# ru1ven/KeypointFusion

Measured on AMD Instinct MI355X. Metric: RGB-D img/sec fwd (B=64, 256x256), higher is better.
Workload: dtype f32; 1 GPU; KPFusion-convnext-tiny, depth+RGB UNet backbones forward, B=64/GPU 256x256 f32 (BASELINE configs[1]); batch_per_gpu=64, global_batch=64, input=256x256, parallelism=dp1 (batch shards, no collective)

## Files before the change

include/kpf.h:

```cpp
#ifndef KPF_H
#define KPF_H

#ifdef __cplusplus
extern "C" {
#endif

#define KPF_OK 0
#define KPF_EINVAL (-1)
#define KPF_ELAUNCH (-2)

#define KPF_DT_F32 0
#define KPF_DT_BF16 1
#define KPF_DT_F16 2
#define KPF_DT_F32_MMA_BF16 8
#define KPF_DT_F32_MMA_F16 9

#define KPF_ACT_RELU 1u
#define KPF_ACT_GELU 2u
#define KPF_RES_ADD 4u
#define KPF_RES_GAMMA 8u
#define KPF_RELU_AFTER_RES 16u
#define KPF_ACT_LEAKY 64u
#define KPF_IN_SPLIT 128u
#define KPF_W_SPLIT 512u
// ... 11 lines not shown
  int OH, OW, N;
  int KH, KW, sh, sw, ph, pw;
  int Kp;
  int out_ld, out_coff;
  int res_ld, res_coff;
  unsigned flags;
  float w_unscale;
  int tile_cfg;
  int groups;
  long w_gstride;
} kpf_conv_desc;

int kpf_conv2d_f32(const kpf_conv_desc* d, const float* in, const float* w, const float* bias,
                   const float* pro_scale, const float* pro_shift, const float* gamma, const float* res,
                   float* out, void* stream);

int kpf_dwconv7_ln_f32(const float* x, const float* w_dw, const float* b_dw, const float* ln_w, const float* ln_b,
                       float* y, int B, int H, int W, int C, float eps, void* stream);

int kpf_convnext_mlp_f32(const float* y, const float* x, const float* w1, const float* b1, const float* w2, const float* b2,
                         const float* gamma, float* out, long M, int C, void* stream);
int kpf_convnext_mlp_supported(int C);
int kpf_convnext_mlp_split_f32(const float* y_split, const float* x, const float* w1_split, const float* b1, float w1_unscale,
                               const float* w2_split_perm, const float* b2, float w2_unscale, const float* gamma, float* out, long M,
                               int C, void* stream);
int kpf_convnext_mlp_split_supported(int C);
int kpf_convnext_mlp_h16(const void* y, const void* x, const void* w1, const float* b1, const void* w2_chunks, const float* b2,
                         const float* gamma, void* out, long M, int C, int dtype, void* stream);
int kpf_convnext_mlp_h16_supported(int C);

// ... 324 lines not shown
int kpf_track_step_f32(const float* joints, const float* center, const float* M, const float* cube, const float* cam_para, const int* pcl_count, int B, int J,
                       int frame_w, int frame_h, float expansion, long long seed_stride, double* bbox, long long* seed, int* lost, float* crop_px,
                       float* frame_px, float* cam_mm, double* bbox_used, int* status, void* stream);

int kpf_prep_annot_u16(const unsigned char* rgb, const unsigned short* depth, const int* frame_index, int F, const float* joints_mm, const float* cam32,
                       const float* center_xyz, const unsigned char* mirror, const double* cube, int B, int J, int Hs, int Ws, int x0, int y0, int H, int W, int S,
                       float* img, float* img_rgb, float* center, float* M, float* cube_out, float* cam_para, double* com, int* bounds, double* M64, float* joint,
                       float* joint_img, double* cam64, void* stream);

int kpf_prep_uncrop_mirror_f32(const float* joints, const float* center, const float* M, const float* cube, const float* cam, const unsigned char* mirror,
                               int frame_w, int B, int J, float* crop_px, float* frame_px, void* stream);

int kpf_conv_num_tile_cfgs(void);

const char* kpf_last_error(void);
#define KPF_ABI_VERSION 23
int kpf_abi_version(void);

#ifdef __cplusplus
}
#endif
#endif
```

keypointfusion_amd/csrc/kpf_conv.hip:

```cpp
#include "kpf_common.h"
#include <stdlib.h>
#include <type_traits>

namespace {

struct ConvArgs {
  const float* in;
  const float* w;
  const float* bias;
  const float* ps;
  const float* pt;
  const float* gamma;
  const float* res;
  float* out;
  int M, N, K, Kp;
  int IH, IW, Cin, in_ld, in_coff;
  int OH, OW, ohow, KH, KW, sh, sw, ph, pw;
  int out_ld, out_coff, res_ld, res_coff;
  const float* zero;
  float w_unscale;
  unsigned flags;
  int tilesN, nblk;
  int vec;
  int dbg;
  int st_policy;
  int skew;
  int groups, g_in, g_out;
  long g_w;
};

__device__ __forceinline__ ConvArgs kpf_group_args(const ConvArgs& a0) {
  ConvArgs a = a0;
  const int g = blockIdx.y;
  a.in_coff += g * a.g_in;
  a.out_coff += g * a.g_out;
  a.res_coff += g * a.g_out;
  a.w += (long)g * a.g_w;
  if (a.bias) a.bias += g * a.g_out;
  return a;
}

__device__ __forceinline__ float gelu_erf(float x) {
  const float z = fabsf(x) * 0.70710678118654752440f;
  const float t = __builtin_amdgcn_rcpf(fmaf(0.3275911f, z, 1.0f));
  float p = fmaf(1.061405429f, t, -1.453152027f);
// ... 26 lines not shown
typedef __attribute__((address_space(3))) void lds_void_t;
typedef __attribute__((address_space(1))) void gbl_void_t;

__device__ __attribute__((aligned(16))) float kpf_zero16[4] = {0.f, 0.f, 0.f, 0.f};

#ifdef KPF_DBG_TIME
__device__ unsigned long long kpf_dbg_t[8 * 8192];
#define KPF_STAMP(i) do { if (threadIdx.x == 0 && blockIdx.x < 8192) { kpf_dbg_t[8 * blockIdx.x + (i)] = __builtin_readcyclecounter(); \
    if ((i) == 0) { kpf_dbg_t[8 * blockIdx.x + 4] = __builtin_amdgcn_s_memrealtime(); kpf_dbg_t[8 * blockIdx.x + 6] = __builtin_amdgcn_s_getreg((4 << 0) | (0 << 6) | (31 << 11)) | ((unsigned long long)__builtin_amdgcn_s_getreg((20 << 0) | (0 << 6) | (3 << 11)) << 32); } \
    if ((i) == 3) kpf_dbg_t[8 * blockIdx.x + 5] = __builtin_amdgcn_s_memrealtime(); } } while (0)
#else
#define KPF_STAMP(i)
#endif
constexpr int BK = 32;

template <int TM, int TN, int WM, int WN, bool IS1X1, bool HAS_PRO, int EPI, int ARITH, int NS>
__device__ __forceinline__ void igemm_body(const ConvArgs& a) {
  constexpr bool SPLIT = ARITH == ARITH_SPLIT || ARITH == ARITH_SPLIT_W;
  constexpr bool H16 = ARITH == ARITH_BF16 || ARITH == ARITH_F16;
  using TH = typename std::conditional<ARITH == ARITH_BF16, bf16_t, f16_t>::type;
  constexpr int BM = 16 * TM * WM;
  constexpr int BN = 16 * TN * WN;
  constexpr int NW = WM * WN;
  constexpr int RPP = 8 * NW;
  constexpr int AP = (BM + RPP - 1) / RPP;
  constexpr int BP = (BN + RPP - 1) / RPP;
  constexpr bool R16 = ARITH == ARITH_R_BF16 || ARITH == ARITH_R_F16;
  constexpr bool WHOLE = NS > 2 || ARITH == ARITH_F32 || R16;
  constexpr int BMR = WHOLE ? AP * RPP : BM;
  constexpr int BNR = WHOLE ? BP * RPP : BN;
  constexpr int TILE = (BMR + BNR) * BK;
  constexpr int CNT = AP + BP;
// ... 45 lines not shown
      riy[p] = oy * a.sh - a.ph;
      rix[p] = ox * a.sw - a.pw;
      pa[p] = a.in + ((long)b * a.IH * a.IW + (long)riy[p] * a.IW + rix[p]) * a.in_ld + a.in_coff;
    } else {
      pa[p] = a.zero;
      riy[p] = -(1 << 20);
      rix[p] = 0;
    }
  }
#pragma unroll
  for (int p = 0; p < BP; ++p) {
    const int n = n0 + lr + RPP * p;
    const int nc = n < a.N ? n : a.N - 1;
    pb[p] = a.w + (long)nc * a.Kp + kc;
  }
  int s_kt = 0, s_tap = 0, s_c = 0;
  const int s_q = IS1X1 ? 0 : BK / a.Cin, s_r = IS1X1 ? 0 : BK - s_q * a.Cin;
  const int s_rcp = IS1X1 ? 0 : (65536 + a.KW - 1) / a.KW;
  if (!IS1X1) {
    s_tap = kc / a.Cin;
    s_c = kc - s_tap * a.Cin;
  }

  auto stage = [&](int kt, int buf) {
    float* As = lds + buf * TILE;
    float* Bs = As + BMR * BK;
    if (IS1X1) {
#pragma unroll
      for (int p = 0; p < AP; ++p)
        if (WHOLE || RPP * p + 8 * wave < BM)
// ... 20 lines not shown
      }
    }
#pragma unroll
    for (int p = 0; p < BP; ++p)
      if (WHOLE || RPP * p + 8 * wave < BN)
        __builtin_amdgcn_global_load_lds((gbl_void_t*)(pb[p] + kt * BK), (lds_void_t*)(Bs + (RPP * p + 8 * wave) * BK), 16, 0, 0);
  };

  const f32x4 zero4 = {0.f, 0.f, 0.f, 0.f};
  f32x4 acc[TN][TM];
#pragma unroll
  for (int i = 0; i < TN; ++i)
#pragma unroll
    for (int j = 0; j < TM; ++j) acc[i][j] = zero4;

  const int nk = a.Kp / BK;
  const int fr = lane & 15;
  const int fg = lane >> 4;
  const int rsw = (fr >> 1) & 7;

  constexpr int EPW = H16 ? 2 : 1;
  float* pro_s = lds + NS * TILE;
  float* pro_t = pro_s + a.Kp * EPW;
  if (NS <= 2) {
    stage(0, 0);
  } else {
#pragma unroll
    for (int t = 0; t < NS - 1; ++t)
      if (t < nk) stage(t, t);
  }
  if (HAS_PRO) {
// ... 22 lines not shown
        const f32x4 tp = *reinterpret_cast<const f32x4*>(pro_t + kk);
#pragma unroll
        for (int j = 0; j < TM; ++j)
#pragma unroll
          for (int e = 0; e < 4; ++e) xf[j][e] = fmaxf(fmaf(xf[j][e], sp[e], tp[e]), 0.f);
      }
    };
    auto mma = [&](int e, const f32x4(&xf)[TM], const f32x4(&wf)[TN]) {
#pragma unroll
      for (int i = 0; i < TN; ++i)
#pragma unroll
        for (int j = 0; j < TM; ++j) acc[i][j] = __builtin_amdgcn_mfma_f32_16x16x4f32(wf[i][e], xf[j][e], acc[i][j], 0, 0, 0);
    };
    f32x4 xa[TM], wa[TN], xb[TM], wb[TN];
    read_frags(0, 0, xa, wa);
    if (nk > 1) stage(1, 1);
    for (int kt = 0; kt + 1 < nk; ++kt) {
      const int cur = kt & 1;
      read_frags(cur, 1, xb, wb);
      prologue(kt, 0, xa);
#pragma unroll
      for (int e = 0; e < 4; ++e) mma(e, xa, wa);
      prologue(kt, 1, xb);
#pragma unroll
      for (int e = 0; e < 3; ++e) mma(e, xb, wb);
      __builtin_amdgcn_sched_barrier(0);
      asm volatile("s_waitcnt vmcnt(0) lgkmcnt(0)" ::: "memory");
      __builtin_amdgcn_s_barrier();
      __builtin_amdgcn_sched_barrier(0);
      read_frags(cur ^ 1, 0, xa, wa);
      stage(kt + 2 < nk ? kt + 2 : nk - 1, cur);
      mma(3, xb, wb);
      __builtin_amdgcn_sched_group_barrier(0x100, TM + TN, 0);
#pragma unroll
      for (int q = 0; q < AP + BP; ++q) {
        __builtin_amdgcn_sched_group_barrier(0x008, (TM * TN) / (AP + BP) > 0 ? (TM * TN) / (AP + BP) : 1, 0);
        __builtin_amdgcn_sched_group_barrier(0x020, 1, 0);
      }
    }
    {
      const int kt = nk - 1, cur = kt & 1;
      read_frags(cur, 1, xb, wb);
      prologue(kt, 0, xa);
#pragma unroll
      for (int e = 0; e < 4; ++e) mma(e, xa, wa);
      prologue(kt, 1, xb);
#pragma unroll
      for (int e = 0; e < 4; ++e) mma(e, xb, wb);
    }
    asm volatile("s_waitcnt vmcnt(0)" ::: "memory");
  } else
  if constexpr (NS > 2 && ARITH == ARITH_SPLIT && !HAS_PRO) {
// ... 233 lines not shown
      __syncthreads();
    }
  }

  KPF_STAMP(2);
  const unsigned fl = a.flags;
  const bool interior = (m0 + BM <= a.M) && (n0 + BN <= a.N) && a.vec && !(fl & KPF_OUT_NCHW);
  if (interior) {
    f32x4 bvv[TN], gvv[TN];
#pragma unroll
    for (int i = 0; i < TN; ++i) {
      const int n = n0 + (wn * TN + i) * 16 + fg * 4;
      bvv[i] = a.bias ? *reinterpret_cast<const f32x4*>(a.bias + n) : zero4;
      gvv[i] = (EPI == EPI_RES && (fl & KPF_RES_GAMMA)) ? *reinterpret_cast<const f32x4*>(a.gamma + n) : zero4;
    }
    constexpr bool HAS_RES = EPI == EPI_RES || EPI == EPI_GGRAD;
    constexpr bool STAGED = H16 && !HAS_RES && TN == 4;
    constexpr int RS = TN * 16 + 8;
    TH* stg = reinterpret_cast<TH*>(lds) + wave * (TM * 16) * RS;
    if constexpr (STAGED) __syncthreads();
    f32x4 rvv[HAS_RES ? TM : 1][TN];
    if (HAS_RES) {
#pragma unroll
      for (int j = 0; j < TM; ++j) {
        const long m = m0 + (wm * TM + j) * 16 + fr;
#pragma unroll
        for (int i = 0; i < TN; ++i) {
          const long o = m * a.res_ld + a.res_coff + n0 + (wn * TN + i) * 16 + fg * 4;
          if constexpr (H16) rvv[j][i] = kpf_ld4(reinterpret_cast<const TH*>(a.res) + o);
          else rvv[j][i] = *reinterpret_cast<const f32x4*>(a.res + o);
        }
// ... 4 lines not shown
      const long m = m0 + (wm * TM + j) * 16 + fr;
#pragma unroll
      for (int i = 0; i < TN; ++i) {
        const int n = n0 + (wn * TN + i) * 16 + fg * 4;
        const f32x4 bv = bvv[i], gv = gvv[i];
        f32x4 v = acc[i][j];
        if (SPLIT) {
#pragma unroll
          for (int e = 0; e < 4; ++e) v[e] *= a.w_unscale;
        }
        if (EPI == EPI_RES) {
#pragma unroll
          for (int e = 0; e < 4; ++e) {
            float y = v[e] + bv[e];
            if (fl & KPF_RES_GAMMA) y *= gv[e];
            y += rvv[HAS_RES ? j : 0][i][e];
            if (fl & KPF_RELU_AFTER_RES) y = fmaxf(y, 0.f);
            v[e] = y;
          }
        } else if (EPI == EPI_GGRAD) {
#pragma unroll
          for (int e = 0; e < 4; ++e) v[e] = (v[e] + bv[e]) * gelu_grad_erf(rvv[HAS_RES ? j : 0][i][e]);
        } else if (EPI == EPI_GELU) {
#pragma unroll
          for (int e = 0; e < 4; ++e) v[e] = gelu_of<ARITH>(v[e] + bv[e]);
        } else if (EPI == EPI_GELU2) {
          f32x4 z;
#pragma unroll
          for (int e = 0; e < 4; ++e) z[e] = v[e] + bv[e];
          if constexpr (H16) kpf_st4(reinterpret_cast<TH*>(const_cast<float*>(a.res)) + m * a.res_ld + a.res_coff + n, z);
          else STORE4(const_cast<float*>(a.res) + m * a.res_ld + a.res_coff + n, z);
// ... 88 lines not shown
        float y = (SPLIT ? acc[i][j][e] * a.w_unscale : acc[i][j][e]) + (a.bias ? a.bias[n + e] : 0.f);
        if (EPI == EPI_GELU) y = gelu_of<ARITH>(y);
        if (EPI == EPI_GELU2) {
          if constexpr (H16) {
            reinterpret_cast<TH*>(const_cast<float*>(a.res))[(long)m * a.res_ld + a.res_coff + n + e] = (TH)y;
            y = (float)(TH)y;
          } else {
            const_cast<float*>(a.res)[(long)m * a.res_ld + a.res_coff + n + e] = y;
          }
          y = gelu_exact_erf(y);
        }
        if (EPI == EPI_LIN && (fl & KPF_ACT_RELU)) y = fmaxf(y, 0.f);
        if (EPI == EPI_LIN && (fl & KPF_ACT_LEAKY)) y = fmaxf(y, 0.01f * y);
        if (EPI == EPI_RES) {
          if (fl & KPF_RES_GAMMA) y *= a.gamma[n + e];
          if constexpr (H16) y += (float)reinterpret_cast<const TH*>(a.res)[(long)m * a.res_ld + a.res_coff + n + e];
          else y += a.res[(long)m * a.res_ld + a.res_coff + n + e];
          if (fl & KPF_RELU_AFTER_RES) y = fmaxf(y, 0.f);
        }
        if (EPI == EPI_GGRAD) {
          if constexpr (H16) y *= gelu_grad_erf((float)reinterpret_cast<const TH*>(a.res)[(long)m * a.res_ld + a.res_coff + n + e]);
          else y *= gelu_grad_erf(a.res[(long)m * a.res_ld + a.res_coff + n + e]);
        }
        if (fl & KPF_OUT_NCHW) {
          a.out[((long)b * a.N + n + e) * a.ohow + pix] = y;
        } else if constexpr (H16) {
          reinterpret_cast<TH*>(a.out)[(long)m * a.out_ld + a.out_coff + n + e] = (TH)y;
        } else if (fl & KPF_OUT_SPLIT) {
          const float yc = __builtin_amdgcn_fmed3f(y, -65504.0f, 65504.0f);
          const _Float16 h = (_Float16)yc;
          _Float16* blk = reinterpret_cast<_Float16*>(a.out + (long)m * a.out_ld + a.out_coff + ((n + e) & ~31)) + ((n + e) & 31);
          blk[0] = h;
          blk[32] = (_Float16)(yc - (float)h);
        } else
          a.out[(long)m * a.out_ld + a.out_coff + n + e] = y;
      }
    }
  }
}

template <int TM, int TN, int WM, int WN, bool IS1X1, bool HAS_PRO, int EPI, int NS>
__global__ __launch_bounds__(64 * WM * WN) void igemm_f32_kernel(const ConvArgs a) {
  igemm_body<TM, TN, WM, WN, IS1X1, HAS_PRO, EPI, ARITH_F32, NS>(kpf_group_args(a));
}
template <int TM, int TN, int WM, int WN, bool IS1X1, int EPI, int ARITH>
__global__ __launch_bounds__(64 * WM * WN) void igemm_r16_kernel(const ConvArgs a) {
  igemm_body<TM, TN, WM, WN, IS1X1, false, EPI, ARITH, 2>(kpf_group_args(a));
}
template <int TM, int TN, int WM, int WN, bool IS1X1, bool HAS_PRO, int EPI, int ARITH, int NS>
__global__ __launch_bounds__(64 * WM * WN) void igemm_split_kernel(const ConvArgs a) {
  igemm_body<TM, TN, WM, WN, IS1X1, HAS_PRO, EPI, ARITH, NS>(kpf_group_args(a));
}
template <int TM, int TN, int WM, int WN, bool IS1X1, bool HAS_PRO, int EPI, int ARITH>
__global__ __launch_bounds__(64 * WM * WN, 4) void igemm_split_occ_kernel(const ConvArgs a) {
  igemm_body<TM, TN, WM, WN, IS1X1, HAS_PRO, EPI, ARITH, 1>(kpf_group_args(a));
}

template <int TM, int TN, int WM, int WN, bool IS1X1, bool HAS_PRO, int EPI, int ARITH, int NS>
// ... 31 lines not shown
  else
    kern = igemm_split_kernel<TM, TN, WM, WN, IS1X1, HAS_PRO, EPI, ARITH, NS>;
  static std::atomic<bool> lds_opt_in[KPF_MAX_DEVICES];
  if (!kpf_raise_lds_limit(reinterpret_cast<const void*>(kern), lds_opt_in)) {
    kpf_set_error("kpf_conv2d_f32: cannot raise the dynamic LDS limit");
    return KPF_ELAUNCH;
  }
  if (lds > 160 * 1024) {
    kpf_set_error("kpf_conv2d_f32: operand prologue too long for LDS (Kp=%d)", a.Kp);
    return KPF_EINVAL;
  }
  hipLaunchKernelGGL(kern, dim3(a.nblk, a.groups > 1 ? a.groups : 1), dim3(64 * WM * WN), lds, st, a);
  return kpf_check_launch("kpf_conv2d_f32");
}

template <int TM, int TN, int WM, int WN, int ARITH, int NS>
int launch_arith(ConvArgs& a, bool is1x1, hipStream_t st) {
  const bool res = a.flags & KPF_RES_ADD, gelu = a.flags & KPF_ACT_GELU;
  if (a.ps) {
    if (!is1x1 || res || gelu || ARITH == ARITH_SPLIT || (NS == 1 && (ARITH == ARITH_BF16 || ARITH == ARITH_F16))) {
      kpf_set_error("kpf_conv2d_f32: the operand prologue is only supported for 1x1 stride-1 convolutions with Cin %% 32 == 0, fp32 activations and a linear/ReLU epilogue");
      return KPF_EINVAL;
    }
    return launch_one<TM, TN, WM, WN, true, true, EPI_LIN, ARITH == ARITH_SPLIT ? ARITH_F32 : ARITH, NS>(a, st);
  }
  if (gelu) {
    if (!is1x1 || res) {
      kpf_set_error("kpf_conv2d_f32: GELU is only supported on 1x1 convolutions (Cin %% 32 == 0) without residual");
      return KPF_EINVAL;
    }
    if (a.flags & KPF_ACT_GELU_SAVE) {
      if constexpr (ARITH == ARITH_F32 && NS == 2) return launch_one<TM, TN, WM, WN, true, false, EPI_GELU2, ARITH, NS>(a, st);
      kpf_set_error("kpf_conv2d_f32: KPF_ACT_GELU_SAVE needs fp32 arithmetic");
// ... 2 lines not shown
    return launch_one<TM, TN, WM, WN, true, false, EPI_GELU, ARITH, NS>(a, st);
  }
  if (a.flags & KPF_RES_GELU_GRAD) {
    if constexpr (ARITH == ARITH_F32 && NS == 2) {
      if (a.KH == 1 && a.KW == 1 && a.sh == 1 && a.sw == 1)
        return is1x1 ? launch_one<TM, TN, WM, WN, true, false, EPI_GGRAD, ARITH, NS>(a, st) : launch_one<TM, TN, WM, WN, false, false, EPI_GGRAD, ARITH, NS>(a, st);
    }
    kpf_set_error("kpf_conv2d_f32: KPF_RES_GELU_GRAD needs a 1x1 stride-1 convolution in fp32 arithmetic");
    return KPF_EINVAL;
  }
  if (is1x1) return res ? launch_one<TM, TN, WM, WN, true, false, EPI_RES, ARITH, NS>(a, st) : launch_one<TM, TN, WM, WN, true, false, EPI_LIN, ARITH, NS>(a, st);
  return res ? launch_one<TM, TN, WM, WN, false, false, EPI_RES, ARITH, NS>(a, st) : launch_one<TM, TN, WM, WN, false, false, EPI_LIN, ARITH, NS>(a, st);
}

template <int TM, int TN, int WM, int WN, int NS_SPLIT = 2>
int launch_cfg(ConvArgs& a, bool is1x1, hipStream_t st) {
  constexpr int BM = 16 * TM * WM, BN = 16 * TN * WN;
  const int tilesM = (a.M + BM - 1) / BM;
  a.tilesN = (a.N + BN - 1) / BN;
  a.nblk = tilesM * a.tilesN;
  static const int stagger = []() { const char* e = getenv("KPF_STAGGER"); return e ? atoi(e) : 0; }();
  const long skew = (long)BM * BN * a.Kp / (128L * 5 * 2048);
  a.skew = a.nblk >= 512 ? (int)(skew < stagger ? skew : stagger) : 0;
  if constexpr ((TM == 4 && TN == 4 && WN == 2 && (WM == 4 || WM == 2)) || (TM == 2 && TN == 4 && WM == 4 && WN == 1)) {
    if ((a.flags & (KPF_MMA_BF16 | KPF_MMA_F16)) && is1x1 && !a.ps && !(a.flags & (KPF_RES_ADD | KPF_ACT_GELU | KPF_IN_SPLIT | KPF_W_SPLIT | KPF_OUT_SPLIT | KPF_OUT_NCHW))) {
      if (a.flags & KPF_MMA_BF16) return launch_one<TM, TN, WM, WN, true, false, EPI_LIN, ARITH_R_BF16, 2>(a, st);
      return launch_one<TM, TN, WM, WN, true, false, EPI_LIN, ARITH_R_F16, 2>(a, st);
    }
  }
  if (a.flags & KPF_IN_SPLIT) return launch_arith<TM, TN, WM, WN, ARITH_SPLIT, NS_SPLIT>(a, is1x1, st);
  if (a.flags & KPF_W_SPLIT) return launch_arith<TM, TN, WM, WN, ARITH_SPLIT_W, NS_SPLIT>(a, is1x1, st);
// ... 560 lines not shown
    case 1: return launch_cfg_h16<4, 3, 2, 2, 2>(a, fast1x1, pointwise, dtype, st);
    case 2: return launch_cfg_h16<2, 4, 4, 1, 2>(a, fast1x1, pointwise, dtype, st);
    case 5: return launch_cfg_h16<2, 4, 2, 2, 2>(a, fast1x1, pointwise, dtype, st);
    case 6: return occ ? launch_cfg_h16<2, 2, 2, 2, 1>(a, fast1x1, pointwise, dtype, st) : launch_cfg_h16<2, 2, 2, 2, 2>(a, fast1x1, pointwise, dtype, st);
    case 8: return launch_cfg_h16<4, 4, 4, 2, 2>(a, fast1x1, pointwise, dtype, st);
    case 20: return launch_cfg_h16<4, 4, 4, 2, 3>(a, fast1x1, pointwise, dtype, st);
    case 21: return launch_cfg_h16<4, 4, 2, 2, 3>(a, fast1x1, pointwise, dtype, st);
    case 22: return launch_cfg_h16<4, 4, 2, 2, 4>(a, fast1x1, pointwise, dtype, st);
    case 26: return launch_cfg_h16<8, 4, 2, 4, 2>(a, fast1x1, pointwise, dtype, st);
    case 41: return launch_cfg_h16<2, 2, 2, 2, 4>(a, fast1x1, pointwise, dtype, st);
    case 44: return launch_cfg_h16<2, 1, 1, 4, 8>(a, fast1x1, pointwise, dtype, st);
    default: return launch_cfg_h16<2, 1, 1, 4, 2>(a, fast1x1, pointwise, dtype, st);
  }
}
#else
extern "C" int kpf_conv2d_f32(const kpf_conv_desc* d, const float* in, const float* w, const float* bias,
                              const float* pro_scale, const float* pro_shift, const float* gamma, const float* res,
                              float* out, void* stream) {
  KPF_REQUIRE(d && in && w && out, "kpf_conv2d_f32: null pointer");
  KPF_REQUIRE(d->B > 0 && d->OH > 0 && d->OW > 0 && d->N > 0 && d->Cin > 0, "kpf_conv2d_f32: empty shape");
  KPF_REQUIRE(d->Cin % 4 == 0 && d->in_ld % 4 == 0 && d->in_coff % 4 == 0,
              "kpf_conv2d_f32: Cin/in_ld/in_coff must be multiples of 4 (got %d/%d/%d)", d->Cin, d->in_ld, d->in_coff);
  KPF_REQUIRE(d->Kp % 32 == 0 && d->Kp >= d->KH * d->KW * d->Cin, "kpf_conv2d_f32: Kp=%d must be a multiple of 32 and >= K=%d",
              d->Kp, d->KH * d->KW * d->Cin);
  KPF_REQUIRE(kpf_aligned16(in) && kpf_aligned16(w) && kpf_aligned16(out), "kpf_conv2d_f32: pointers must be 16-byte aligned");
  const unsigned fl = d->flags;
  if (!(fl & KPF_OUT_NCHW))
    KPF_REQUIRE(d->out_coff >= 0 && d->out_coff + d->N <= d->out_ld, "kpf_conv2d_f32: bad output slice ld=%d coff=%d N=%d",
                d->out_ld, d->out_coff, d->N);
  if (fl & KPF_RES_ADD)
    KPF_REQUIRE(res && kpf_aligned16(res) && d->res_coff >= 0 && d->res_coff + d->N <= d->res_ld, "kpf_conv2d_f32: bad residual");
  if (fl & KPF_RES_GAMMA) KPF_REQUIRE(gamma && (fl & KPF_RES_ADD), "kpf_conv2d_f32: RES_GAMMA needs gamma and RES_ADD");
  KPF_REQUIRE((pro_scale == nullptr) == (pro_shift == nullptr), "kpf_conv2d_f32: prologue needs both scale and shift");
  KPF_REQUIRE(((fl & KPF_ACT_RELU) != 0) + ((fl & KPF_ACT_GELU) != 0) + ((fl & KPF_ACT_LEAKY) != 0) <= 1, "kpf_conv2d_f32: one activation only");
  KPF_REQUIRE(!((fl & KPF_RES_ADD) && (fl & (KPF_ACT_RELU | KPF_ACT_GELU | KPF_ACT_LEAKY))), "kpf_conv2d_f32: activation before a residual add is not supported");
  KPF_REQUIRE(!((fl & KPF_ACT_LEAKY) && pro_scale), "kpf_conv2d_f32: LeakyReLU is not combined with an operand prologue");
  KPF_REQUIRE(!(fl & KPF_RELU_AFTER_RES) || (fl & KPF_RES_ADD), "kpf_conv2d_f32: RELU_AFTER_RES needs RES_ADD");
  KPF_REQUIRE(!(fl & KPF_RES_GELU_GRAD) || ((fl & KPF_RES_ADD) && !(fl & (KPF_RES_GAMMA | KPF_RELU_AFTER_RES | KPF_OUT_NCHW))), "kpf_conv2d_f32: RES_GELU_GRAD goes with RES_ADD alone");
  KPF_REQUIRE(!(fl & KPF_ACT_GELU_SAVE) || ((fl & KPF_ACT_GELU) && !(fl & (KPF_RES_ADD | KPF_OUT_NCHW)) && res && kpf_aligned16(res) && d->res_coff >= 0 && d->res_coff + d->N <= d->res_ld),
              "kpf_conv2d_f32: ACT_GELU_SAVE goes with ACT_GELU and a second output buffer in the res slot (res_ld / res_coff describe it)");
  KPF_REQUIRE((long)d->B * d->OH * d->OW < (1l << 31) && (long)d->B * d->IH * d->IW < (1l << 31), "kpf_conv2d_f32: too many pixels");

  ConvArgs a;
  a.in = in; a.w = w; a.bias = bias; a.ps = pro_scale; a.pt = pro_shift; a.gamma = gamma; a.res = res; a.out = out;
  a.M = d->B * d->OH * d->OW; a.N = d->N; a.K = d->KH * d->KW * d->Cin; a.Kp = d->Kp;
  a.IH = d->IH; a.IW = d->IW; a.Cin = d->Cin; a.in_ld = d->in_ld; a.in_coff = d->in_coff;
  a.OH = d->OH; a.OW = d->OW; a.ohow = d->OH * d->OW; a.KH = d->KH; a.KW = d->KW;
  a.sh = d->sh; a.sw = d->sw; a.ph = d->ph; a.pw = d->pw;
  a.out_ld = d->out_ld; a.out_coff = d->out_coff; a.res_ld = d->res_ld; a.res_coff = d->res_coff;
  {
    static const float* zero_of_dev[64] = {nullptr};
    int dev = 0;
    if (hipGetDevice(&dev) != hipSuccess || dev < 0 || dev >= 64) dev = 0;
    if (!zero_of_dev[dev]) {
      void* p = nullptr;
      if (hipGetSymbolAddress(&p, HIP_SYMBOL(kpf_zero16)) != hipSuccess || !p) {
        kpf_set_error("kpf_conv2d_f32: cannot resolve the zero page");
        return KPF_ELAUNCH;
// ... 73 lines not shown
    case 8: return launch_cfg<4, 4, 4, 2>(a, is1x1, st);
    case 9: return launch_cfg<4, 4, 4, 2, 3>(a, is1x1, st);
    case 10: return launch_cfg<4, 4, 2, 2>(a, is1x1, st);
    case 11: return launch_cfg<4, 3, 2, 2>(a, is1x1, st);
    case 12: return launch_cfg<2, 4, 4, 1, 3>(a, is1x1, st);
    case 13: return launch_cfg<4, 4, 2, 2, 1>(a, is1x1, st);
    case 14: return launch_cfg<4, 3, 2, 2, 1>(a, is1x1, st);
    case 15: return launch_cfg<2, 4, 4, 1, 1>(a, is1x1, st);
    case 16: return launch_cfg<2, 2, 2, 2, 1>(a, is1x1, st);
    case 17: return launch_cfg<4, 6, 2, 2>(a, is1x1, st);
    default: return launch_cfg<2, 1, 1, 4>(a, is1x1, st);
  }
#endif
}

extern "C" int kpf_conv_num_tile_cfgs(void) { return KPF_NUM_TILE_CFGS; }
#endif

#ifdef KPF_DBG_TIME
extern "C" int kpf_dbg_read(unsigned long long* host, int n) {
  return hipMemcpyFromSymbol(host, HIP_SYMBOL(kpf_dbg_t), sizeof(unsigned long long) * n) == hipSuccess ? 0 : -1;
}
extern "C" int kpf_dbg_clear(void) {
  static unsigned long long z[8 * 8192];
  return hipMemcpyToSymbol(HIP_SYMBOL(kpf_dbg_t), z, sizeof(z)) == hipSuccess ? 0 : -1;
}
#endif
```

keypointfusion_amd/engine.py:

```python
import ctypes as C
import math

import torch

from . import lib as L
from .packs import ConvGeom, Pack, Packed16, PackedConv, split_pack
from .spec import CONVNEXT, parse_net

BN_EPS = 1e-5
FORCE_UNFUSED_MLP = bool(int(__import__("os").environ.get("KPF_UNFUSED_MLP", "0")))
GEMM_MODE = __import__("os").environ.get("KPF_GEMM", "f32")
assert GEMM_MODE in ("split", "f32"), "KPF_GEMM must be 'split' or 'f32'"
F16_MAX = 65504.0
AUTOTUNE = bool(int(__import__("os").environ.get("KPF_AUTOTUNE", "0")))
_TILE_RULES = {tuple(int(v) for v in r.split("=")[0].split(":")): int(r.split("=")[1]) + 1 for r in __import__("os").environ.get("KPF_TILE_RULES", "").split(",") if r}


PROFILE = None
FORCE_TILE = 0


def _launch(kernel, flops, nbytes, shape, fn):
    if PROFILE is None:
        return fn()
# ... 107 lines not shown
        if cfg is None and PROFILE is None and not torch.cuda.is_current_stream_capturing():
            cfg = pc.tuned[key] = _autotune(lib, d, x, w, pc, gamma, res, optr, flags)
        d.tile_cfg = cfg or 0
    if _TILE_RULES and not AUTOTUNE:
        d.tile_cfg = _TILE_RULES.get((M, g.N, g.K, g.KH), 0)
    if FORCE_TILE:
        d.tile_cfg = FORCE_TILE
    nbytes = 4.0 * (x.B * d.IH * d.IW * g.Cin + g.N * g.K + M * g.N * (2 if res is not None else 1))
    ng = max(1, d.groups)
    _launch("igemm_split_kernel" if flags & (L.KPF_IN_SPLIT | L.KPF_W_SPLIT) else "igemm_f32_kernel", g.flops(M) * ng, nbytes * ng, (M, g.N, g.K, g.KH, g.KW),
            lambda: L.check(lib.kpf_conv2d_f32(C.byref(d), _ptr(x.buf), _ptr(w), _ptr(pc.b), _ptr(pc.ps), _ptr(pc.pt), _ptr(gamma),
                                               _ptr(res.buf if res is not None else None), _ptr(optr), _stream()), "kpf_conv2d_f32"))
    return out


def _autotune(lib, d, x, w, pc, gamma, res, optr, flags):
    ncfg = int(lib.kpf_conv_num_tile_cfgs())
    split = bool(flags & (L.KPF_IN_SPLIT | L.KPF_W_SPLIT))
    cands = [i for i in range(ncfg) if split or i < 9 or i == 17]
    out_t = optr
    if res is not None and res.buf.data_ptr() == optr.data_ptr():
        out_t = torch.empty_like(optr)
    args = (_ptr(x.buf), _ptr(w), _ptr(pc.b), _ptr(pc.ps), _ptr(pc.pt), _ptr(gamma), _ptr(res.buf if res is not None else None), _ptr(out_t), _stream())
    torch.cuda.synchronize()
    best, best_t = 0, float("inf")
    for c in cands:
        d.tile_cfg = c + 1
        if lib.kpf_conv2d_f32(C.byref(d), *args) != 0:
            continue
        e0, e1 = torch.cuda.Event(enable_timing=True), torch.cuda.Event(enable_timing=True)
# ... 68 lines not shown

class ResidualPlan:

    def __init__(self, sd, p, device, pack=None, launch=None):
        P = pack or (lambda w, b, **k: PackedConv(w, b, device, **k))
        self.launch = launch or conv
        cin = sd[p + ".conv1.conv.weight"].shape[1]
        cout = sd[p + ".conv3.conv.weight"].shape[0]
        self.cin, self.cout = cin, cout
        self.c1 = P(sd[p + ".conv1.conv.weight"], sd[p + ".conv1.conv.bias"], fold_bn=bn_scale_shift(sd, p + ".bn2"), prologue=bn_scale_shift(sd, p + ".bn1"))
        self.c2 = P(sd[p + ".conv2.conv.weight"], sd[p + ".conv2.conv.bias"], pad=1, fold_bn=bn_scale_shift(sd, p + ".bn3"))
        self.c3 = P(sd[p + ".conv3.conv.weight"], sd[p + ".conv3.conv.bias"])
        self.skip = P(sd[p + ".skip_layer.conv.weight"], sd[p + ".skip_layer.conv.bias"]) if cin != cout else None

    def __call__(self, x, out=None):
        conv = self.launch
        h = conv(self.c1, x, flags=L.KPF_ACT_RELU)
        h = conv(self.c2, h, flags=L.KPF_ACT_RELU)
        if out is None:
            out = Act.empty(x.B, x.H, x.W, self.cout, x.buf.device, x.buf.dtype)
        if self.skip is not None:
            conv(self.skip, x, out=out)
            return conv(self.c3, h, out=out, res=out)
        return conv(self.c3, h, out=out, res=x)

    def flops(self, M):
        f = self.c1.flops(M) + self.c2.flops(M) + self.c3.flops(M)
        return f + (self.skip.flops(M) if self.skip else 0)


class ConvNeXtBlockPlan:

    def __init__(self, sd, p, device):
        c = sd[p + ".gamma"].numel()
        self.C = c
        self.wdw = sd[p + ".dwconv.weight"].detach().float().reshape(c, 49).t().contiguous().to(device)
        self.bdw = sd[p + ".dwconv.bias"].detach().float().to(device)
        self.lnw = sd[p + ".norm.weight"].detach().float().to(device)
        self.lnb = sd[p + ".norm.bias"].detach().float().to(device)
# ... 443 lines not shown
```

keypointfusion_amd/lib.py:

```python
import ctypes as C
import os

_HERE = os.path.dirname(os.path.abspath(__file__))
LIB_PATH = os.environ.get("KPF_LIB_PATH") or os.path.join(_HERE, "libkpf_hip.so")

KPF_ACT_RELU = 1
KPF_ACT_GELU = 2
KPF_RES_ADD = 4
KPF_RES_GAMMA = 8
KPF_RELU_AFTER_RES = 16
KPF_RES_GELU_GRAD = 1024
KPF_ACT_GELU_SAVE = 2048
KPF_PRO_LN = 4096
KPF_DT_F32_MMA_BF16, KPF_DT_F32_MMA_F16 = 8, 9
KPF_MMA_BF16, KPF_MMA_F16 = 8192, 16384
KPF_OUT_NCHW = 32
KPF_ACT_LEAKY = 64
KPF_IN_SPLIT = 128
KPF_OUT_SPLIT = 256
KPF_W_SPLIT = 512
KPF_DT_F32, KPF_DT_BF16, KPF_DT_F16 = 0, 1, 2
ABI_VERSION = 23


class ConvDesc(C.Structure):
    _fields_ = [(n, C.c_int) for n in (
        "B", "IH", "IW", "Cin", "in_ld", "in_coff", "OH", "OW", "N", "KH", "KW", "sh", "sw", "ph", "pw", "Kp",
        "out_ld", "out_coff", "res_ld", "res_coff")] + [("flags", C.c_uint), ("w_unscale", C.c_float), ("tile_cfg", C.c_int), ("groups", C.c_int), ("w_gstride", C.c_long)]


class PackDesc(C.Structure):
    _fields_ = [("src", C.c_void_p), ("dst", C.c_void_p)] + [(n, C.c_int) for n in (
        "N", "Cin", "KH", "KW", "mode", "n_pad", "Kp", "rows", "src_dtype", "dst_dtype", "first_block", "reserved")]


class AdamwDesc(C.Structure):
    _fields_ = [("p", C.c_void_p), ("g", C.c_void_p), ("m", C.c_void_p), ("v", C.c_void_p), ("n", C.c_long), ("first_block", C.c_int), ("reserved", C.c_int)]
# ... 10 lines not shown
class WgradReduceDesc(C.Structure):
    _fields_ = [("part", C.c_void_p), ("dbpart", C.c_void_p), ("dw", C.c_void_p), ("db", C.c_void_p), ("g_ws", C.c_long)] + [
        (n, C.c_int) for n in "S N K Cin KHW nkb ndb groups Cin_out N_out kind first_block".split()]


class WgradPlan(C.Structure):
    _fields_ = [(n, C.c_int) for n in "family vn vk tiles_n tiles_k S sps writes_dw".split()] + [("ws_floats", C.c_long)]


KPF_WGRAD_FAMILY = ("f32", "r16", "direct", "h16s", "h16")
KPF_WGRAD_FORM = {"f32_2x2": 1, "f32_2x4": 2, "f32_4x2": 3, "f32_4x4": 4, "h16s": 5, "h16": 6}

_P = C.c_void_p
_SIGS = {
    "kpf_conv2d_f32": [C.POINTER(ConvDesc), _P, _P, _P, _P, _P, _P, _P, _P, _P],
    "kpf_dwconv7_ln_f32": [_P, _P, _P, _P, _P, _P, C.c_int, C.c_int, C.c_int, C.c_int, C.c_float, _P],
    "kpf_layernorm_f32": [_P, _P, _P, _P, C.c_long, C.c_int, C.c_float, _P],
    "kpf_layernorm_split_f32": [_P, _P, _P, _P, C.c_long, C.c_int, C.c_float, _P],
    "kpf_dwconv7_ln_split_f32": [_P, _P, _P, _P, _P, _P, C.c_int, C.c_int, C.c_int, C.c_int, C.c_float, _P],
    "kpf_upsample2x_f32": [_P, _P, C.c_int, C.c_int, C.c_int, C.c_int, C.c_int, C.c_int, _P],
    "kpf_nchw_to_nhwc_f32": [_P, _P, C.c_int, C.c_int, C.c_int, C.c_int, C.c_int, _P],
    "kpf_nhwc_to_nchw_f32": [_P, _P, C.c_int, C.c_int, C.c_int, C.c_int, C.c_int, C.c_int, _P],
    "kpf_maxpool3x3s2_f32": [_P, _P, C.c_int, C.c_int, C.c_int, C.c_int, _P],
    "kpf_inv3x3_f32": [_P, _P, C.c_int, C.c_int, _P],
    "kpf_offset2joint_f32": [_P] * 8 + [C.c_int, C.c_int, C.c_int, C.c_float, C.c_int, C.c_int, _P],
    "kpf_img2pcl_top4_f32": [_P] * 9 + [C.c_int] * 6 + [_P],
    "kpf_point_assemble_f32": [_P] * 9 + [C.c_int, C.c_int, C.c_int, C.c_float, _P],
    "kpf_softmax_pool_f32": [_P, _P, _P, _P, C.c_int, C.c_int, _P],
    "kpf_ball_group_f32": [_P, _P, _P, _P, C.c_int, _P, _P, C.c_int, C.c_int, C.c_float, C.c_float, C.c_float, _P],
    "kpf_group_max_f32": [_P, _P, C.c_long, C.c_int, C.c_int, C.c_int, C.c_int, _P],
# ... 180 lines not shown
```

Measured before the change: 3533 img/s.

## Fuse residual skip 1x1 conv and final 1x1 conv into one paired GEMM

Adds a paired fp32 1x1 implicit-GEMM kernel. It first runs the skip-layer GEMM over its K range, holds that result plus its bias in registers, then runs the main conv's K range and adds the held values in the epilogue. This replaces two launches and the round trip of writing the skip result to the output and reading it back as a residual. The cost is extra register pressure from the held accumulators, limited by a launch-bounds occupancy hint of 2, and a fallback to two launches when the estimated register count is too high. Residual blocks with a projection skip use the paired kernel by default when shapes allow.

Result: no change. 3563 img/s (median of 6 runs) (+0.9%).

```diff
diff --git a/include/kpf.h b/include/kpf.h
--- a/include/kpf.h
+++ b/include/kpf.h
@@ -49,6 +49,9 @@
 int kpf_conv2d_f32(const kpf_conv_desc* d, const float* in, const float* w, const float* bias,
                    const float* pro_scale, const float* pro_shift, const float* gamma, const float* res,
                    float* out, void* stream);
+
+int kpf_conv2d_pair_f32(const kpf_conv_desc* d, const float* in, const float* w, const float* bias, const kpf_conv_desc* d2, const float* in2,
+                        const float* w2, const float* bias2, float* out, void* stream);
 
 int kpf_dwconv7_ln_f32(const float* x, const float* w_dw, const float* b_dw, const float* ln_w, const float* ln_b,
                        float* y, int B, int H, int W, int C, float eps, void* stream);
@@ -403,7 +406,7 @@
 int kpf_conv_num_tile_cfgs(void);
 
 const char* kpf_last_error(void);
-#define KPF_ABI_VERSION 23
+#define KPF_ABI_VERSION 24
 int kpf_abi_version(void);
 
 #ifdef __cplusplus
diff --git a/keypointfusion_amd/csrc/kpf_conv.hip b/keypointfusion_amd/csrc/kpf_conv.hip
--- a/keypointfusion_amd/csrc/kpf_conv.hip
+++ b/keypointfusion_amd/csrc/kpf_conv.hip
@@ -29,6 +29,13 @@
   long g_w;
 };
 
+struct PairArgs : ConvArgs {
+  const float* in2;
+  const float* w2;
+  const float* bias2;
+  int Kp2, in2_ld, in2_coff;
+};
+
 __device__ __forceinline__ ConvArgs kpf_group_args(const ConvArgs& a0) {
   ConvArgs a = a0;
   const int g = blockIdx.y;
@@ -85,8 +92,9 @@
 #endif
 constexpr int BK = 32;
 
-template <int TM, int TN, int WM, int WN, bool IS1X1, bool HAS_PRO, int EPI, int ARITH, int NS>
-__device__ __forceinline__ void igemm_body(const ConvArgs& a) {
+template <int TM, int TN, int WM, int WN, bool IS1X1, bool HAS_PRO, int EPI, int ARITH, int NS, bool PAIR = false, class Args = ConvArgs>
+__device__ __forceinline__ void igemm_body(const Args& a) {
+  static_assert(!PAIR || (ARITH == ARITH_F32 && NS == 2 && IS1X1 && !HAS_PRO && EPI == EPI_RES), "the pair form exists for the fp32 two-stage dense 1x1 GEMM only");
   constexpr bool SPLIT = ARITH == ARITH_SPLIT || ARITH == ARITH_SPLIT_W;
   constexpr bool H16 = ARITH == ARITH_BF16 || ARITH == ARITH_F16;
   using TH = typename std::conditional<ARITH == ARITH_BF16, bf16_t, f16_t>::type;
@@ -162,6 +170,38 @@
     const int nc = n < a.N ? n : a.N - 1;
     pb[p] = a.w + (long)nc * a.Kp + kc;
   }
+  [[maybe_unused]] auto set_phase = [&](const float* in, int ld, int coff, const float* w, int kp, int t0) {
+#pragma unroll
+    for (int p = 0; p < AP; ++p) {
+      const int m = m0 + lr + RPP * p;
+      const int mc = m < a.M ? m : a.M - 1;
+      pa[p] = in + ((long)mc * ld + coff + kc - (long)t0 * BK);
+    }
+#pragma unroll
+    for (int p = 0; p < BP; ++p) {
+      const int n = n0 + lr + RPP * p;
+      const int nc = n < a.N ? n : a.N - 1;
+      pb[p] = w + ((long)nc * kp + kc - (long)t0 * BK);
+    }
+  };
+  int nk1 = 0;
+  f32x4 held[PAIR ? TN : 1][PAIR ? TM : 1];
+  f32x4 b2v[PAIR ? TN : 1];
+  if constexpr (PAIR) {
+    nk1 = a.Kp2 / BK;
+#pragma unroll
+    for (int i = 0; i < TN; ++i)
+#pragma unroll
+      for (int j = 0; j < TM; ++j) held[i][j] = f32x4{0.f, 0.f, 0.f, 0.f};
+    set_phase(a.in2, a.in2_ld, a.in2_coff, a.w2, a.Kp2, 0);
+#pragma unroll
+    for (int i = 0; i < TN; ++i)
+#pragma unroll
+      for (int e = 0; e < 4; ++e) {
+        const int n = n0 + (wave / WM * TN + i) * 16 + (lane >> 4) * 4 + e;
+        b2v[i][e] = a.bias2 ? a.bias2[n < a.N ? n : a.N - 1] : 0.f;
+      }
+  }
   int s_kt = 0, s_tap = 0, s_c = 0;
   const int s_q = IS1X1 ? 0 : BK / a.Cin, s_r = IS1X1 ? 0 : BK - s_q * a.Cin;
   const int s_rcp = IS1X1 ? 0 : (65536 + a.KW - 1) / a.KW;
@@ -212,7 +252,7 @@
 #pragma unroll
     for (int j = 0; j < TM; ++j) acc[i][j] = zero4;
 
-  const int nk = a.Kp / BK;
+  const int nk = a.Kp / BK + nk1;
   const int fr = lane & 15;
   const int fg = lane >> 4;
   const int rsw = (fr >> 1) & 7;
@@ -265,9 +305,13 @@
     };
     f32x4 xa[TM], wa[TN], xb[TM], wb[TN];
     read_frags(0, 0, xa, wa);
+    if constexpr (PAIR)
+      if (nk1 == 1) set_phase(a.in, a.in_ld, a.in_coff, a.w, a.Kp, nk1);
     if (nk > 1) stage(1, 1);
     for (int kt = 0; kt + 1 < nk; ++kt) {
       const int cur = kt & 1;
+      if constexpr (PAIR)
+        if (kt + 2 == nk1) set_phase(a.in, a.in_ld, a.in_coff, a.w, a.Kp, nk1);
       read_frags(cur, 1, xb, wb);
       prologue(kt, 0, xa);
 #pragma unroll
@@ -287,6 +331,18 @@
       for (int q = 0; q < AP + BP; ++q) {
         __builtin_amdgcn_sched_group_barrier(0x008, (TM * TN) / (AP + BP) > 0 ? (TM * TN) / (AP + BP) : 1, 0);
         __builtin_amdgcn_sched_group_barrier(0x020, 1, 0);
+      }
+      if constexpr (PAIR) {
+        if (kt + 1 == nk1) {
+#pragma unroll
+          for (int i = 0; i < TN; ++i)
+#pragma unroll
+            for (int j = 0; j < TM; ++j) {
+#pragma unroll
+              for (int e = 0; e < 4; ++e) held[i][j][e] = acc[i][j][e] + b2v[i][e];
+              acc[i][j] = zero4;
+            }
+        }
       }
     }
     {
@@ -550,7 +606,7 @@
       bvv[i] = a.bias ? *reinterpret_cast<const f32x4*>(a.bias + n) : zero4;
       gvv[i] = (EPI == EPI_RES && (fl & KPF_RES_GAMMA)) ? *reinterpret_cast<const f32x4*>(a.gamma + n) : zero4;
     }
-    constexpr bool HAS_RES = EPI == EPI_RES || EPI == EPI_GGRAD;
+    constexpr bool HAS_RES = (EPI == EPI_RES || EPI == EPI_GGRAD) && !PAIR;
     constexpr bool STAGED = H16 && !HAS_RES && TN == 4;
     constexpr int RS = TN * 16 + 8;
     TH* stg = reinterpret_cast<TH*>(lds) + wave * (TM * 16) * RS;
@@ -585,7 +641,8 @@
           for (int e = 0; e < 4; ++e) {
             float y = v[e] + bv[e];
             if (fl & KPF_RES_GAMMA) y *= gv[e];
-            y += rvv[HAS_RES ? j : 0][i][e];
+            if constexpr (PAIR) y += held[i][j][e];
+            else y += rvv[HAS_RES ? j : 0][i][e];
             if (fl & KPF_RELU_AFTER_RES) y = fmaxf(y, 0.f);
             v[e] = y;
           }
@@ -704,7 +761,8 @@
         if (EPI == EPI_LIN && (fl & KPF_ACT_LEAKY)) y = fmaxf(y, 0.01f * y);
         if (EPI == EPI_RES) {
           if (fl & KPF_RES_GAMMA) y *= a.gamma[n + e];
-          if constexpr (H16) y += (float)reinterpret_cast<const TH*>(a.res)[(long)m * a.res_ld + a.res_coff + n + e];
+          if constexpr (PAIR) y += held[i][j][e];
+          else if constexpr (H16) y += (float)reinterpret_cast<const TH*>(a.res)[(long)m * a.res_ld + a.res_coff + n + e];
           else y += a.res[(long)m * a.res_ld + a.res_coff + n + e];
           if (fl & KPF_RELU_AFTER_RES) y = fmaxf(y, 0.f);
         }
@@ -732,6 +790,10 @@
 template <int TM, int TN, int WM, int WN, bool IS1X1, bool HAS_PRO, int EPI, int NS>
 __global__ __launch_bounds__(64 * WM * WN) void igemm_f32_kernel(const ConvArgs a) {
   igemm_body<TM, TN, WM, WN, IS1X1, HAS_PRO, EPI, ARITH_F32, NS>(kpf_group_args(a));
+}
+template <int TM, int TN, int WM, int WN>
+__global__ __launch_bounds__(64 * WM * WN, 2) void igemm_f32_kernel(const PairArgs a) {
+  igemm_body<TM, TN, WM, WN, true, false, EPI_RES, ARITH_F32, 2, true>(a);
 }
 template <int TM, int TN, int WM, int WN, bool IS1X1, int EPI, int ARITH>
 __global__ __launch_bounds__(64 * WM * WN) void igemm_r16_kernel(const ConvArgs a) {
@@ -793,9 +855,39 @@
   return kpf_check_launch("kpf_conv2d_f32");
 }
 
+template <int TM, int TN, int WM, int WN>
+int launch_pair(const PairArgs& a, hipStream_t st) {
+  constexpr int NW = WM * WN, AP = (16 * TM * WM + 8 * NW - 1) / (8 * NW), BP = (16 * TN * WN + 8 * NW - 1) / (8 * NW);
+  if constexpr (8 * TM * TN + 8 * (TM + TN) + 2 * (AP + BP) + 4 * TN > 220) {
+    ConvArgs s = a;
+    s.in = a.in2; s.w = a.w2; s.bias = a.bias2; s.Kp = s.K = s.Cin = a.Kp2; s.in_ld = a.in2_ld; s.in_coff = a.in2_coff;
+    s.res = nullptr; s.flags = 0;
+    const int rc = launch_one<TM, TN, WM, WN, true, false, EPI_LIN, ARITH_F32, 2>(s, st);
+    if (rc != KPF_OK) return rc;
+    ConvArgs m = a;
+    m.res = a.out; m.res_ld = a.out_ld; m.res_coff = a.out_coff;
+    return launch_one<TM, TN, WM, WN, true, false, EPI_RES, ARITH_F32, 2>(m, st);
+  } else {
+    constexpr int BM = 16 * TM * WM, BN = 16 * TN * WN, RPP = 8 * WM * WN;
+    constexpr int BMR = (BM + RPP - 1) / RPP * RPP, BNR = (BN + RPP - 1) / RPP * RPP;
+    const size_t lds = (size_t)(2 * (BMR + BNR) * BK) * sizeof(float);
+    void (*kern)(const PairArgs) = igemm_f32_kernel<TM, TN, WM, WN>;
+    static std::atomic<bool> lds_opt_in[KPF_MAX_DEVICES];
+    if (!kpf_raise_lds_limit(reinterpret_cast<const void*>(kern), lds_opt_in)) {
+      kpf_set_error("kpf_conv2d_pair_f32: cannot raise the dynamic LDS limit");
+      return KPF_ELAUNCH;
+    }
+    hipLaunchKernelGGL(kern, dim3(a.nblk), dim3(64 * WM * WN), lds, st, a);
+    return kpf_check_launch("kpf_conv2d_pair_f32");
+  }
+}
+
 template <int TM, int TN, int WM, int WN, int ARITH, int NS>
-int launch_arith(ConvArgs& a, bool is1x1, hipStream_t st) {
+int launch_arith(PairArgs& a, bool is1x1, hipStream_t st) {
   const bool res = a.flags & KPF_RES_ADD, gelu = a.flags & KPF_ACT_GELU;
+  if constexpr (ARITH == ARITH_F32 && NS == 2) {
+    if (a.Kp2 > 0) return launch_pair<TM, TN, WM, WN>(a, st);
+  }
   if (a.ps) {
     if (!is1x1 || res || gelu || ARITH == ARITH_SPLIT || (NS == 1 && (ARITH == ARITH_BF16 || ARITH == ARITH_F16))) {
       kpf_set_error("kpf_conv2d_f32: the operand prologue is only supported for 1x1 stride-1 convolutions with Cin %% 32 == 0, fp32 activations and a linear/ReLU epilogue");
@@ -828,7 +920,7 @@
 }
 
 template <int TM, int TN, int WM, int WN, int NS_SPLIT = 2>
-int launch_cfg(ConvArgs& a, bool is1x1, hipStream_t st) {
+int launch_cfg(PairArgs& a, bool is1x1, hipStream_t st) {
   constexpr int BM = 16 * TM * WM, BN = 16 * TN * WN;
   const int tilesM = (a.M + BM - 1) / BM;
   a.tilesN = (a.N + BN - 1) / BN;
@@ -1419,9 +1511,23 @@
   }
 }
 #else
+struct PairSecond {
+  const float* in;
+  const float* w;
+  const float* bias;
+  int Kp, in_ld, in_coff;
+};
+static int conv2d_f32_run(const kpf_conv_desc* d, const float* in, const float* w, const float* bias, const float* pro_scale, const float* pro_shift,
+                          const float* gamma, const float* res, float* out, void* stream, const PairSecond* second);
+
 extern "C" int kpf_conv2d_f32(const kpf_conv_desc* d, const float* in, const float* w, const float* bias,
                               const float* pro_scale, const float* pro_shift, const float* gamma, const float* res,
                               float* out, void* stream) {
+  return conv2d_f32_run(d, in, w, bias, pro_scale, pro_shift, gamma, res, out, stream, nullptr);
+}
+
+static int conv2d_f32_run(const kpf_conv_desc* d, const float* in, const float* w, const float* bias, const float* pro_scale, const float* pro_shift,
+                          const float* gamma, const float* res, float* out, void* stream, const PairSecond* second) {
   KPF_REQUIRE(d && in && w && out, "kpf_conv2d_f32: null pointer");
   KPF_REQUIRE(d->B > 0 && d->OH > 0 && d->OW > 0 && d->N > 0 && d->Cin > 0, "kpf_conv2d_f32: empty shape");
   KPF_REQUIRE(d->Cin % 4 == 0 && d->in_ld % 4 == 0 && d->in_coff % 4 == 0,
@@ -1446,7 +1552,9 @@
               "kpf_conv2d_f32: ACT_GELU_SAVE goes with ACT_GELU and a second output buffer in the res slot (res_ld / res_coff describe it)");
   KPF_REQUIRE((long)d->B * d->OH * d->OW < (1l << 31) && (long)d->B * d->IH * d->IW < (1l << 31), "kpf_conv2d_f32: too many pixels");
 
-  ConvArgs a;
+  PairArgs a;
+  a.in2 = a.w2 = a.bias2 = nullptr; a.Kp2 = a.in2_ld = a.in2_coff = 0;
+  if (second) { a.in2 = second->in; a.w2 = second->w; a.bias2 = second->bias; a.Kp2 = second->Kp; a.in2_ld = second->in_ld; a.in2_coff = second->in_coff; }
   a.in = in; a.w = w; a.bias = bias; a.ps = pro_scale; a.pt = pro_shift; a.gamma = gamma; a.res = res; a.out = out;
   a.M = d->B * d->OH * d->OW; a.N = d->N; a.K = d->KH * d->KW * d->Cin; a.Kp = d->Kp;
   a.IH = d->IH; a.IW = d->IW; a.Cin = d->Cin; a.in_ld = d->in_ld; a.in_coff = d->in_coff;
@@ -1550,6 +1658,43 @@
 #endif
 }
 
+extern "C" int kpf_conv2d_pair_f32(const kpf_conv_desc* d, const float* in, const float* w, const float* bias, const kpf_conv_desc* d2, const float* in2,
+                                   const float* w2, const float* bias2, float* out, void* stream) {
+  KPF_REQUIRE(d && d2 && in && w && in2 && w2 && out, "kpf_conv2d_pair_f32: null pointer");
+  KPF_REQUIRE(d->B > 0 && d->OH > 0 && d->OW > 0 && d->N > 0, "kpf_conv2d_pair_f32: empty shape");
+  const kpf_conv_desc* ds[2] = {d, d2};
+  for (int i = 0; i < 2; ++i) {
+    const kpf_conv_desc* q = ds[i];
+    const char* who = i ? "second" : "main";
+    KPF_REQUIRE(q->KH == 1 && q->KW == 1, "kpf_conv2d_pair_f32: the %s layer is not a 1x1 convolution (%d x %d taps)", who, q->KH, q->KW);
+    KPF_REQUIRE(q->sh == 1 && q->sw == 1 && q->ph == 0 && q->pw == 0 && q->IH == q->OH && q->IW == q->OW,
+                "kpf_conv2d_pair_f32: the %s layer has a stride or padding (dense stride-1 layers only)", who);
+    KPF_REQUIRE(q->Cin > 0 && q->Cin % 32 == 0, "kpf_conv2d_pair_f32: the %s layer's Cin %% 32 != 0 (Cin=%d)", who, q->Cin);
+    KPF_REQUIRE(q->Kp == q->Cin, "kpf_conv2d_pair_f32: the %s layer needs Kp == Cin (Kp=%d, Cin=%d)", who, q->Kp, q->Cin);
+    KPF_REQUIRE(q->in_ld % 4 == 0 && q->in_coff % 4 == 0 && q->in_coff >= 0 && q->in_coff + q->Cin <= q->in_ld,
+                "kpf_conv2d_pair_f32: bad input slice of the %s layer (ld=%d coff=%d Cin=%d)", who, q->in_ld, q->in_coff, q->Cin);
+    const unsigned f = q->flags & ~KPF_RES_ADD;
+    KPF_REQUIRE(!(f & (KPF_IN_SPLIT | KPF_W_SPLIT | KPF_OUT_SPLIT)), "kpf_conv2d_pair_f32: split operand flags on the %s layer", who);
+    KPF_REQUIRE(!(f & (KPF_MMA_BF16 | KPF_MMA_F16)), "kpf_conv2d_pair_f32: 16-bit product flags (MMA_BF16 / MMA_F16) on the %s layer", who);
+    KPF_REQUIRE(!(f & (KPF_ACT_GELU | KPF_ACT_GELU_SAVE | KPF_RES_GELU_GRAD)), "kpf_conv2d_pair_f32: GELU flags on the %s layer", who);
+    KPF_REQUIRE(!(f & KPF_OUT_NCHW), "kpf_conv2d_pair_f32: OUT_NCHW on the %s layer", who);
+    KPF_REQUIRE(!(f & KPF_RES_GAMMA), "kpf_conv2d_pair_f32: RES_GAMMA on the %s layer", who);
+    KPF_REQUIRE(!(f & KPF_RELU_AFTER_RES), "kpf_conv2d_pair_f32: RELU_AFTER_RES on the %s layer", who);
+    KPF_REQUIRE(!(f & (KPF_ACT_RELU | KPF_ACT_LEAKY | KPF_PRO_LN)), "kpf_conv2d_pair_f32: an activation or prologue flag on the %s layer", who);
+    KPF_REQUIRE(q->groups <= 1, "kpf_conv2d_pair_f32: groups = %d on the %s layer (one convolution each)", q->groups, who);
+  }
+  KPF_REQUIRE(d->B == d2->B && d->OH == d2->OH && d->OW == d2->OW, "kpf_conv2d_pair_f32: the layers' pixel counts (M) differ: %d x %d x %d against %d x %d x %d",
+              d->B, d->OH, d->OW, d2->B, d2->OH, d2->OW);
+  KPF_REQUIRE(d->N == d2->N, "kpf_conv2d_pair_f32: the layers' output widths (N) differ: %d against %d", d->N, d2->N);
+  KPF_REQUIRE(d->out_ld == d2->out_ld && d->out_coff == d2->out_coff, "kpf_conv2d_pair_f32: the layers name different output slices (one `out`)");
+  KPF_REQUIRE(kpf_aligned16(in2) && kpf_aligned16(w2), "kpf_conv2d_pair_f32: pointers must be 16-byte aligned");
+  kpf_conv_desc m = *d;
+  m.flags = KPF_RES_ADD;
+  m.res_ld = d->out_ld; m.res_coff = d->out_coff;
+  const PairSecond sec = {in2, w2, bias2, d2->Kp, d2->in_ld, d2->in_coff};
+  return conv2d_f32_run(&m, in, w, bias, nullptr, nullptr, nullptr, out, out, stream, &sec);
+}
+
 extern "C" int kpf_conv_num_tile_cfgs(void) { return KPF_NUM_TILE_CFGS; }
 #endif
 
diff --git a/keypointfusion_amd/engine.py b/keypointfusion_amd/engine.py
--- a/keypointfusion_amd/engine.py
+++ b/keypointfusion_amd/engine.py
@@ -1,5 +1,6 @@
 import ctypes as C
 import math
+import os
 
 import torch
 
@@ -145,6 +146,28 @@
     return out
 
 
+def _pair_ok(pc, x):
+    g = pc.geom
+    return (g.KH == g.KW == g.sh == g.sw == g.merge == 1 and g.ph == g.pw == 0 and g.Cin % 32 == 0 and g.Kp == g.Cin and pc.ps is None and not pc.groups
+            and not x.split and x.buf.dtype == torch.float32 and not (GEMM_MODE == "split" and pc.split_allowed) and not AUTOTUNE and not _TILE_RULES)
+
+
+def conv_pair(pc, x, pc2, x2, out):
+    lib = L.load()
+    d, out, optr, _, (M, _, _) = conv_desc(pc, x, pc.geom.Kp, out)
+    d2, _, _, _, (M2, _, _) = conv_desc(pc2, x2, pc2.geom.Kp, out)
+    assert M == M2
+    out.split = False
+    if FORCE_TILE:
+        d.tile_cfg = FORCE_TILE
+    g, g2 = pc.geom, pc2.geom
+    nbytes = 4.0 * (M * (g.Cin + g2.Cin) + g.N * (g.K + g2.K) + M * g.N)
+    _launch("igemm_f32_kernel", g.flops(M) + g2.flops(M), nbytes, (M, g.N, g.K + g2.K, 1, 1),
+            lambda: L.check(lib.kpf_conv2d_pair_f32(C.byref(d), _ptr(x.buf), _ptr(pc.w), _ptr(pc.b), C.byref(d2), _ptr(x2.buf), _ptr(pc2.w), _ptr(pc2.b),
+                                                    _ptr(optr), _stream()), "kpf_conv2d_pair_f32"))
+    return out
+
+
 def _autotune(lib, d, x, w, pc, gamma, res, optr, flags):
     ncfg = int(lib.kpf_conv_num_tile_cfgs())
     split = bool(flags & (L.KPF_IN_SPLIT | L.KPF_W_SPLIT))
@@ -243,15 +266,17 @@
         self.skip = P(sd[p + ".skip_layer.conv.weight"], sd[p + ".skip_layer.conv.bias"]) if cin != cout else None
 
     def __call__(self, x, out=None):
-        conv = self.launch
-        h = conv(self.c1, x, flags=L.KPF_ACT_RELU)
-        h = conv(self.c2, h, flags=L.KPF_ACT_RELU)
+        run = self.launch
+        h = run(self.c1, x, flags=L.KPF_ACT_RELU)
+        h = run(self.c2, h, flags=L.KPF_ACT_RELU)
         if out is None:
             out = Act.empty(x.B, x.H, x.W, self.cout, x.buf.device, x.buf.dtype)
         if self.skip is not None:
-            conv(self.skip, x, out=out)
-            return conv(self.c3, h, out=out, res=out)
-        return conv(self.c3, h, out=out, res=x)
+            if run is conv and _pair_ok(self.c3, h) and _pair_ok(self.skip, x) and os.environ.get("KPF_RES_PAIR", "1") != "0":
+                return conv_pair(self.c3, h, self.skip, x, out)
+            run(self.skip, x, out=out)
+            return run(self.c3, h, out=out, res=out)
+        return run(self.c3, h, out=out, res=x)
 
     def flops(self, M):
         f = self.c1.flops(M) + self.c2.flops(M) + self.c3.flops(M)
diff --git a/keypointfusion_amd/lib.py b/keypointfusion_amd/lib.py
--- a/keypointfusion_amd/lib.py
+++ b/keypointfusion_amd/lib.py
@@ -20,7 +20,7 @@
 KPF_OUT_SPLIT = 256
 KPF_W_SPLIT = 512
 KPF_DT_F32, KPF_DT_BF16, KPF_DT_F16 = 0, 1, 2
-ABI_VERSION = 23
+ABI_VERSION = 24
 
 
 class ConvDesc(C.Structure):
@@ -61,6 +61,7 @@
 _P = C.c_void_p
 _SIGS = {
     "kpf_conv2d_f32": [C.POINTER(ConvDesc), _P, _P, _P, _P, _P, _P, _P, _P, _P],
+    "kpf_conv2d_pair_f32": [C.POINTER(ConvDesc), _P, _P, _P, C.POINTER(ConvDesc), _P, _P, _P, _P, _P],
     "kpf_dwconv7_ln_f32": [_P, _P, _P, _P, _P, _P, C.c_int, C.c_int, C.c_int, C.c_int, C.c_float, _P],
     "kpf_layernorm_f32": [_P, _P, _P, _P, C.c_long, C.c_int, C.c_float, _P],
     "kpf_layernorm_split_f32": [_P, _P, _P, _P, C.c_long, C.c_int, C.c_float, _P],
```
